# CVMethods/gabor_color_image_segmentation

Measured on AMD Instinct MI355X. Metric: Mpix/s segmented (Gabor+k-means), 481x321x3 batch, higher is better.
Workload: dtype i8; 1 GPU; batch 64/GPU synthetic 481x321x3 uint8 (seed 0), 4-scale x 6-orientation Gabor bank ksize 13 on a 2-level octave pyramid, k=8, n_iter=10; codebook=global, global_batch=64, parallelism=dp1 (images sharded, int64 centroid all-reduce)

## Files before the change

### gabor_color_image_segmentation_amd/_lib.py

```python
from __future__ import annotations

import ctypes as C
import os

_HERE = os.path.dirname(os.path.abspath(__file__))
LIB_PATH = os.environ.get("GCS_LIB_PATH") or os.path.join(_HERE, "csrc", "libgcs.so")

ABI_VERSION = 18
K_MAX = 16

_vp, _i, _sz = C.c_void_p, C.c_int, C.c_size_t

SIGNATURES = {
    "gcs_abi_version": (_i, []),
    "gcs_last_error": (C.c_char_p, []),
    "gcs_bank_packed_bytes": (_sz, [_i, _i]),
    "gcs_bank_bias_count": (_sz, [_i, _i]),
    "gcs_bank_pack": (_i, [_vp, _i, _i, _i, _vp, _vp]),
    "gcs_feature_slab_bytes": (_sz, [_i, _i, _i, _i, _i]),
    "gcs_feature_pass_bytes": (_sz, [_i, _i, _i, _i, _i]),
    "gcs_label_slab_bytes": (_sz, [_i, _i, _i]),
    "gcs_kmeans_parts_per_image": (_sz, [_i, _i, _i]),
    "gcs_kmeans_partial_bytes": (_sz, [_i, _i, _i, _i, _i]),
    "gcs_gabor_workspace_bytes": (_sz, [_i, _i, _i, _i]),
    "gcs_gabor_features": (_i, [_vp, _i, _i, _i, _vp, _vp, _i, _i, _i, _i, _vp, _vp, _vp]),
    "gcs_features_unpack": (_i, [_vp, _i, _i, _i, _i, _i, _vp, _vp]),
    "gcs_kmeans_init": (_i, [_vp, _i, _i, _i, _i, _i, _i, _i, _vp, _vp]),
    "gcs_features_gather": (_i, [_vp, _i, _i, _i, _i, _i, _i, _vp, _vp, _vp]),
    "gcs_kmeans_assign_accumulate": (_i, [_vp, _vp, _i, _i, _i, _i, _i, _i, _i, _i, _i, _i, _vp, _vp, _vp]),
    "gcs_kmeans_assign_raster": (_i, [_vp, _vp, _i, _i, _i, _i, _i, _i, _i, _i, _vp, _i, _vp, _vp]),
    "gcs_kmeans_reduce": (_i, [_vp, _i, _i, _i, _i, _i, _i, _vp, _vp]),
    "gcs_kmeans_finalize": (_i, [_vp, _i, _i, _i, _vp, _vp]),
    "gcs_kmeans_reduce_finalize": (_i, [_vp, _i, _i, _i, _i, _i, _i, _vp, _vp, _vp]),
    "gcs_download": (_i, [_vp, _vp, _sz, _vp]),
    "gcs_labels_widen": (_i, [_vp, _i, _i, _i, _vp, _vp]),
    "gcs_selftest_isqrt": (_i, [C.c_uint, _vp, _vp]),
    "gcs_selftest_native_parts": (_i, [_i, _i, _i]),
    "gcs_device_cu_count": (_i, []),
    "gcs_boundary_scratch_bytes": (_sz, [_i, _i, _i]),
    "gcs_boundary_counts": (_i, [_vp, _vp, _i, _i, _i, _vp, _vp, _vp]),
    "gcs_region_counts": (_i, [_vp, _vp, _i, _i, _i, _i, _i, _vp, _vp, _vp, _vp]),
    "gcs_boundary_batch_scratch_bytes": (_sz, [_i, _i, _i, _i]),
    "gcs_boundary_counts_batch": (_i, [_vp, _vp, _vp, _i, _i, _i, _i, _vp, _vp, _vp]),
    "gcs_region_counts_batch": (_i, [_vp, _vp, _vp, _i, _i, _i, _i, _i, _i, _i, _vp, _vp, _vp, _vp]),
    "gcs_region_counts_batch_u8": (_i, [_vp, _vp, _vp, _i, _i, _i, _i, _i, _i, _i, _vp, _vp, _vp, _vp]),
    "gcs_region_reduce": (_i, [_vp, _vp, _vp, _i, _i, _i, _vp, _vp, _vp]),
    "gcs_score_batch_resident": (_i, [_vp, _vp, _vp, _vp, _i, _vp, _vp, _i, _i, _i, _i, _i, _i, _i, _vp, _vp, _vp, _vp, _vp, _vp,
                                      _vp, _vp, _vp]),
# ... 49 lines not shown
```

### gabor_color_image_segmentation_amd/csrc/common.h

```cpp
#pragma once
#include <hip/hip_runtime.h>
#include <stdint.h>
#include <stdio.h>
#include <string.h>

#include "gcs.h"

typedef int v2i __attribute__((ext_vector_type(2)));
typedef int v4i __attribute__((ext_vector_type(4)));
typedef int v16i __attribute__((ext_vector_type(16)));

int gcs_fail(int code, const char *msg);
int gcs_hip_fail(hipError_t e, const char *what);
#define GCS_CHECK_LAUNCH(what)                               \
    do {                                                     \
        hipError_t e_ = hipGetLastError();                   \
        if (e_ != hipSuccess) return gcs_hip_fail(e_, what); \
    } while (0)

int gcs_cu_count();

static inline int round_up(int a, int m) { return (a + m - 1) / m * m; }
static inline int mtiles(int F) { return (F + 3) / 4; }

// ... 163 lines not shown
    const unsigned gi = slot % g, second = gi >= h ? 1u : 0u;
    byte = (slot / g) * h + gi - second * h;
    shift = 4 * (int)second;
}
__device__ __forceinline__ unsigned gcs_slab_value(const unsigned char *feats, const GcsLayout &lo, int b, int r, int y, int x) {
    if (!lo.split) return *reinterpret_cast<const uint16_t *>(feats + gcs_slab_offset(lo, b, r, y, x)) ^ 0x8080u;
    const unsigned char *img = feats + (size_t)b * lo.img_bytes;
    const unsigned slot = gcs_split_slot(lo, r, y, x);
    unsigned nb;
    int sh;
    gcs_split_nibble(gcs_level_of_plane(lo, r), slot, nb, sh);
    const unsigned lo8 = img[slot] ^ 0x80u, mid = (img[lo.mid_off + nb] >> sh) & 15u, top = (img[lo.top_off + nb] >> sh) & 15u;
    return lo8 | (mid << 8) | (top << 12);
}

constexpr int KP_PCH = 16;
__host__ __device__ __forceinline__ int partial_chunks(int row_len) { return (row_len + KP_PCH - 1) / KP_PCH; }
__device__ __forceinline__ size_t partial_index(int per_image, int b, int part, int parts, int nb, int i, int row_len) {
    const size_t rows = per_image ? (size_t)parts : (size_t)nb * parts;
    const size_t row = per_image ? (size_t)part : (size_t)b * parts + part;
    const size_t set = per_image ? (size_t)b : 0;
    return ((set * partial_chunks(row_len) + (size_t)(i / KP_PCH)) * rows + row) * KP_PCH + (size_t)(i % KP_PCH);
}
```

### gabor_color_image_segmentation_amd/csrc/kmeans.hip

```cpp
#include "common.h"
#include <type_traits>

#define LAYOUT_OR_FAIL(lo, who)                                        \
    GcsLayout lo;                                                      \
    if (B <= 0 || !gcs_make_layout(H, W, n_scales, n_orient, &lo))     \
        return gcs_fail(GCS_EINVAL, who ": bad shape or bank")

__global__ void kmeans_init_kernel(const unsigned char *__restrict__ feats, GcsLayout lo, int k,
                                   uint16_t *__restrict__ cent) {
    const int set = blockIdx.x;
    const long P = (long)lo.H * lo.W;
    for (int i = threadIdx.x; i < k * lo.D; i += blockDim.x) {
        const int j = i / lo.D, d = i % lo.D;
        const long p = ((2L * j + 1) * P) / (2L * k);
        const int y = (int)(p / lo.W), x = (int)(p % lo.W);
        cent[((size_t)set * k + j) * lo.D + d] = (uint16_t)gcs_slab_value(feats, lo, set, gcs_plane_of_logical(lo, d), y, x);
    }
}

extern "C" int gcs_kmeans_init(const uint16_t *feats, int B, int H, int W, int n_scales, int n_orient, int k,
                               int n_sets, uint16_t *cent, gcs_stream_t stream) {
    if (!feats || !cent) return gcs_fail(GCS_EINVAL, "gcs_kmeans_init: NULL pointer");
    LAYOUT_OR_FAIL(lo, "gcs_kmeans_init");
    if (k < 1 || k > GCS_K_MAX) return gcs_fail(GCS_EINVAL, "gcs_kmeans_init: k must be in 1..16");
// ... 205 lines not shown
    } while (0)
#define KP_PHASE_STORE                                                                                           \
    do {                                                                                                         \
        const int wg_ = (int)(blockIdx.y * gridDim.x + blockIdx.x);                                              \
        if (lane == 0 && wg_ < 1024) {                                                                           \
            for (int k_ = 0; k_ < 6; ++k_) g_kp_phases[(wg_ * 4 + (wid & 3)) * 8 + k_] = kp_ph[k_];             \
            g_kp_phases[(wg_ * 4 + (wid & 3)) * 8 + 6] = kp_tiles;                                               \
        }                                                                                                        \
    } while (0)
#else
#define KP_PHASE_DECL
#define KP_PHASE(k)
#define KP_PHASE_STORE
#endif

template <int KT, int NST, int DSTEPS, int WAVES, bool SPLIT = false, int L0T = 0>
__global__ __launch_bounds__(64 * WAVES, (WAVES == 8 ? 2
                                          : DSTEPS == KP_DSTEPS_NARROW && KT == 1 && NST <= (SPLIT ? 3 : 6) ? GCS_KP_WAVES
                                          : DSTEPS == KP_DSTEPS_NARROW ? 2 : 1)) void kmeans_pass_mfma_kernel(
    const unsigned char *__restrict__ feats, const uint16_t *__restrict__ cent, GcsLayout lo, int K, int per_image,
    int parts, int reverse, int row_lo, int row_hi, uint64_t *__restrict__ partials, void *__restrict__ raster,
    int raster_u8, int nt_flag) {
    constexpr int KP_ROWS = 16 * DSTEPS, KP_DSTEPS = DSTEPS, KP_NT = 2 * DSTEPS;
    constexpr int NTHR = 64 * WAVES;
    constexpr int NT_OWN = WAVES == 8 ? (KP_NT + 1) / 2 : KP_NT;
    constexpr int KP_COARSE = DSTEPS == KP_DSTEPS_NARROW ? 40 * 32 + 64 : 104 * 32 + 64;
    __shared__ __attribute__((aligned(16))) unsigned char s_tile[KP_ROWS * KP_PITCH];
    __shared__ __attribute__((aligned(16))) unsigned char s_coarse[KP_COARSE];
    __shared__ __attribute__((aligned(16))) unsigned char s_lab[KP_TP];
    __shared__ long long s_const[16];
    constexpr int KP_FLAGS = 320;
    __shared__ unsigned char s_flag[SPLIT ? KP_FLAGS : 4];
    static_assert(!SPLIT || (DSTEPS == KP_DSTEPS_NARROW && WAVES == 4), "the split slab is the narrow pass's");

    const bool do_acc = partials != nullptr;
    const int tid = threadIdx.x, lane = tid & 63;
    const int wid = tid >> 6;
    const int wave = wid & 3;
    const int half = wid >> 2;
    const int b = blockIdx.y, part = blockIdx.x;
    const int D = lo.D;
    const uint16_t *cset = cent + (size_t)(per_image ? b : 0) * K * D;
    const int ntiles = lo.ntiles;
    const int nimg = per_image ? 1 : (int)gridDim.y;
    const int G = parts * nimg, g = per_image ? part : b * parts + part;
    const int nlist = ntiles * nimg;
    const unsigned char *fb = feats + (size_t)(per_image ? b : 0) * lo.img_bytes;

    uint16_t *cs = reinterpret_cast<uint16_t *>(s_tile);
    for (int i = tid; i < 8 * KT * KP_ROWS; i += NTHR) {
        const int j = i / KP_ROWS, r = i % KP_ROWS;
        int e = 0;
        if (r >= lo.row0[0] && r < lo.row0[0] + lo.DL[0]) e = kp_logical_of<0>(lo, r - lo.row0[0]);
        if (lo.n_levels > 1 && r >= lo.row0[1] && r < lo.row0[1] + lo.DL[1]) e = kp_logical_of<1>(lo, r - lo.row0[1]);
        if (lo.n_levels > 2 && r >= lo.row0[2] && r < lo.row0[2] + lo.DL[2]) e = kp_logical_of<2>(lo, r - lo.row0[2]);
        if (lo.n_levels > 3 && r >= lo.row0[3] && r < lo.row0[3] + lo.DL[3]) e = kp_logical_of<3>(lo, r - lo.row0[3]);
        cs[i] = (j < K && r < D) ? (uint16_t)(cset[j * D + e] ^ 0x8080u) : (uint16_t)0;
    }
    if constexpr (SPLIT) {
        for (int it = tid; it < KP_FLAGS; it += NTHR) {
            const long long lt = (long long)g + (long long)it * G;
            unsigned char f = 0;
            if (lt < nlist) {
                const int T = reverse ? nlist - 1 - (int)lt : (int)lt;
// ... 539 lines not shown
            } else {
                bx -= dr;
                by -= dq;
                if (bx < 0) { bx += lo.bx_n; --by; }
            }
        }
        KP_PHASE(4);
        __syncthreads();
        KP_PHASE(5);
#ifdef GCS_KP_PHASES
        ++kp_tiles;
#endif
    }
    KP_PHASE_STORE;

    if (!do_acc) return;
    if constexpr (UPD2) {
        constexpr int RW2 = 16 * DSTEPS;
        int *red = reinterpret_cast<int *>(s_tile);
        static_assert(4 * 16 * RW2 * 4 <= KP_ROWS * KP_PITCH, "fold buffer exceeds the tile buffer");
#pragma unroll
        for (int pt = 0; pt < DSTEPS; ++pt)
#pragma unroll
            for (int e = 0; e < 4; ++e) red[(wave * 16 + 4 * ug + e) * RW2 + 16 * pt + un] = accu[pt][e];
        __syncthreads();
        const int D1 = D + 1;
        auto folded = [&](int j, int bb, int plane) {
            int sm_ = 0;
#pragma unroll
            for (int w = 0; w < 4; ++w) sm_ += red[(w * 16 + 2 * j + bb) * RW2 + plane];
            return -(long long)sm_ / 128;
        };
        for (int i = tid; i < K * D1; i += NTHR) {
            const int j = i / D1, e = i % D1;
            const long long nj = folded(j, 0, D);
            long long out = nj;
            if (e < D) {
                const int c = e / lo.F, f = e - c * lo.F;
                int pe = kp_plane_on_level<0>(lo, c, f);
                { const int q = kp_plane_on_level<1>(lo, c, f); pe = q >= 0 ? q : pe; }
                { const int q = kp_plane_on_level<2>(lo, c, f); pe = q >= 0 ? q : pe; }
                { const int q = kp_plane_on_level<3>(lo, c, f); pe = q >= 0 ? q : pe; }
                out = (folded(j, 0, pe) + 128 * nj) + 256 * (folded(j, 1, pe) + 128 * nj);
            }
            partials[partial_index(per_image, b, part, parts, (int)gridDim.y, i, K * D1)] = (uint64_t)out;
        }
    }
    if constexpr (!UPD2) {
    constexpr int RW = KP_NT * 16;
    int *red = reinterpret_cast<int *>(s_tile);
    static_assert(4 * 16 * RW * 4 <= KP_ROWS * KP_PITCH, "fold buffer exceeds the tile buffer");
#pragma unroll
    for (int nti = 0; nti < NT_OWN; ++nti) {
        const int nt = WAVES == 8 ? half * NT_OWN + nti : nti;
        if (nt < KP_NT)
#pragma unroll
            for (int e = 0; e < 4; ++e) red[(wave * 16 + 4 * ug + e) * RW + 16 * nt + un] = accu[nti][e];
    }
    __syncthreads();
// ... 538 lines not shown
    if (B > 65535) return gcs_fail(GCS_EINVAL, "gcs_kmeans_assign_accumulate: B too large for one launch");
    if ((long long)B * lo.ntiles > 0x1fffffffLL)
        return gcs_fail(GCS_EINVAL, "gcs_kmeans_assign_accumulate: batch too large for one launch");
    if (k < 1 || k > GCS_K_MAX) return gcs_fail(GCS_EINVAL, "gcs_kmeans_assign_accumulate: k must be in 1..16");
    if (n_sets != 1 && n_sets != B)
        return gcs_fail(GCS_EINVAL, "gcs_kmeans_assign_accumulate: n_sets must be 1 or B");
    const int D = lo.D;
    if (D < 16 * KP_DSTEPS_WIDE) {
        const int parts = (int)gcs_kmeans_parts_per_image(B, H, W);
        void *lab_out = raster ? raster : static_cast<void *>(labels);
        const int lab_u8 = raster ? raster_u8 : 1;
        const int nt_flag = 0;
#define GCS_KP_LAUNCHW(KT_, NST_, DS_, WV_)                                                                              \
    hipLaunchKernelGGL((kmeans_pass_mfma_kernel<KT_, NST_, DS_, WV_>), dim3(parts, B), dim3(64 * WV_), 0, stream,         \
                       reinterpret_cast<const unsigned char *>(feats), cent, lo, k, n_sets == B ? 1 : 0, parts,          \
                       reverse ? 1 : 0, row_lo, row_hi, partials, lab_out, lab_u8, nt_flag)
#define GCS_KP_LAUNCH(KT_, NST_, DS_) GCS_KP_LAUNCHW(KT_, NST_, DS_, 4)
        const int nchunk = lo.tile_bytes / 16;
        const int nst = (nchunk + 255) / 256;
        if (lo.split) {
            const int rounds = ((lo.S >> 4) + 255) / 256;
            const int nt_limit = kp_nt_limit(lo, B, n_sets, lo.tile_bytes / 4 * 3);
            if ((unsigned long long)lo.img_bytes >= (1ull << 32))
                return gcs_fail(GCS_EINVAL, "gcs_kmeans_assign_accumulate: image too large for the split slab's pass");
#define GCS_KP_LAUNCHS(KT_, NR_, ...)                                                                                          \
    hipLaunchKernelGGL((kmeans_pass_mfma_kernel<KT_, NR_, KP_DSTEPS_NARROW, 4, true __VA_OPT__(,) __VA_ARGS__>), dim3(parts, B), dim3(256), 0, stream, \
                       reinterpret_cast<const unsigned char *>(feats), cent, lo, k, n_sets == B ? 1 : 0, parts,             \
                       reverse ? 1 : 0, row_lo, row_hi, partials, lab_out, lab_u8, nt_limit)
            if (k <= 8 && rounds <= 3 && lo.DL[0] >= 32) { GCS_KP_LAUNCHS(1, 3, 2); }
            else if (k <= 8 && rounds <= 3) { GCS_KP_LAUNCHS(1, 3); }
            else if (k <= 8) { GCS_KP_LAUNCHS(1, 5); }
            else { GCS_KP_LAUNCHS(2, 5); }
#undef GCS_KP_LAUNCHS
        } else if (D < 16 * KP_DSTEPS_NARROW) {
            if (k <= 8) {
                if (nst <= 3) { GCS_KP_LAUNCH(1, 3, KP_DSTEPS_NARROW); }
                else if (nst <= 6) { GCS_KP_LAUNCH(1, 6, KP_DSTEPS_NARROW); }
                else if (nst <= 9) { GCS_KP_LAUNCH(1, 9, KP_DSTEPS_NARROW); }
                else { GCS_KP_LAUNCH(1, 10, KP_DSTEPS_NARROW); }
            } else {
                if (nst <= 6) { GCS_KP_LAUNCH(2, 6, KP_DSTEPS_NARROW); }
                else { GCS_KP_LAUNCH(2, 10, KP_DSTEPS_NARROW); }
            }
// ... 57 lines not shown
                                            int reverse, uint8_t *labels, uint64_t *partials, gcs_stream_t stream) {
    if (!labels && !partials)
        return gcs_fail(GCS_EINVAL, "gcs_kmeans_assign_accumulate: NULL pointer (labels and partials may not both be NULL)");
    return lloyd_pass(feats, cent, B, H, W, n_scales, n_orient, k, n_sets, row_lo, row_hi, reverse, labels, partials, nullptr, 0,
                      stream);
}

extern "C" int gcs_kmeans_assign_raster(const uint16_t *feats, const uint16_t *cent, int B, int H, int W, int n_scales,
                                        int n_orient, int k, int n_sets, int reverse, void *out, int out_u8,
                                        uint8_t *scratch_labels, gcs_stream_t stream) {
    if (!out) return gcs_fail(GCS_EINVAL, "gcs_kmeans_assign_raster: NULL pointer");
    return lloyd_pass(feats, cent, B, H, W, n_scales, n_orient, k, n_sets, 0, H, reverse, scratch_labels, nullptr, out,
                      out_u8 ? 1 : 0, stream);
}

template <bool FIN, int RG>
__global__ __launch_bounds__(16 * RG) void kmeans_reduce_kernel(const uint64_t *__restrict__ partials,
                                                             int rows_per_set, int row_len, int D1,
                                                             long long *__restrict__ sums,
                                                             uint16_t *__restrict__ cent) {
    __shared__ unsigned long long sm_s[RG][KP_PCH], sm_c[RG][KP_PCH];
    const int set = blockIdx.y, chunk = blockIdx.x, t = threadIdx.x;
    const int e16 = t & (KP_PCH - 1), rg = t >> 4;
    const int nch = partial_chunks(row_len);
    const int e = chunk * KP_PCH + e16;
    const int ee = e < row_len ? e : row_len - 1;
    const int j = ee / D1, d = ee - j * D1;
    const int ec = j * D1 + (D1 - 1);
    const uint64_t *p = partials + (((size_t)set * nch + chunk) * rows_per_set) * KP_PCH + (ee - chunk * KP_PCH);
    const uint64_t *pc = partials + (((size_t)set * nch + ec / KP_PCH) * rows_per_set) * KP_PCH + ec % KP_PCH;
// ... 134 lines not shown
```

### gabor_color_image_segmentation_amd/segmenter.py

```python
from __future__ import annotations

import math
import os

import numpy as np

from . import _lib
from .bank import GaborBank, check_color_weight, make_bank, smoothing_taps

_SLAB_BUDGET = 16 << 30
_GRAPH_MAX_PIXELS = 1 << 20


class DebugSwitches:

    def __init__(self, spec=""):
        self.no_reverse = self.no_graph = self.force_collectives = False
        self.slab_candidates = None
        for item in filter(None, (x.strip() for x in spec.split(","))):
            name, _, val = item.partition("=")
            if name == "slab_candidates" and val.isdigit():
                self.slab_candidates = int(val)
            elif name in ("no_reverse", "no_graph", "force_collectives") and not val:
                setattr(self, name, True)
# ... 112 lines not shown
        packed = np.zeros(self.lib.gcs_bank_packed_bytes(ns, no), np.int8)
        bias = np.zeros(self.lib.gcs_bank_bias_count(ns, no), np.int32)
        tapq = np.ascontiguousarray(bank.tapq, np.int16)
        _lib.check(self.lib.gcs_bank_pack(tapq.ctypes.data, ns, no, bank.ksize, packed.ctypes.data,
                                          bias.ctypes.data), "gcs_bank_pack")
        self.packed = torch.from_numpy(packed).to(self.device)
        self.bias = torch.from_numpy(bias).to(self.device)
        self._gabor_ws = None
        self.chroma_gain = _check_chroma_gain(chroma_gain)
        self.smoothing = _check_smoothing(smoothing, bank)
        self._smooth_ws = self.smooth_taps = self.smooth_radius = None
        if self.smoothing > 0:
            taps, radius = smoothing_taps(self.smoothing, ns, no, bank.f_max, bank.ratio)
            self.smooth_taps = torch.from_numpy(taps).to(self.device)
            self.smooth_radius = torch.from_numpy(radius).to(self.device)

    def empty_bytes(self, n):
        return self.torch.empty(int(n), dtype=self.torch.uint8, device=self.device)

    def feature_slab(self, b, h, w):
        return self.empty_bytes(self.lib.gcs_feature_slab_bytes(b, h, w, *self._bk))

    def label_slab(self, b, h, w):
        return self.empty_bytes(self.lib.gcs_label_slab_bytes(b, h, w))

    def partial_slab(self, b, h, w, k):
        return self.empty_bytes(self.lib.gcs_kmeans_partial_bytes(b, h, w, self.bank.n_features, k))

    def _stream(self):
        return self.torch.cuda.current_stream(self.device).cuda_stream

    def _check_dev(self, *tensors):
        for t in tensors:
            if t.device != self.device:
                raise ValueError(f"tensor on {t.device}, this Segmenter's kernels run on {self.device}")

    def gabor_scratch(self, b, h, w):
        return self.empty_bytes(self.lib.gcs_gabor_workspace_bytes(b, h, w, self.bank.n_scales))

    @_on_device
    def gabor_features(self, imgs, feats, scratch=None):
        b, h, w, _ = imgs.shape
# ... 43 lines not shown
                   "gcs_smooth_features")

    @_on_device
    def features_unpack(self, feats, b, h, w):
        d = self.bank.n_features
        out = self.torch.empty((b, d, h, w), dtype=self.torch.int16, device=self.device)
        _lib.check(self.lib.gcs_features_unpack(feats.data_ptr(), b, h, w, *self._bk, out.data_ptr(),
                                                self._stream()), "gcs_features_unpack")
        return out

    @_on_device
    def kmeans_init(self, feats, b, h, w, k, n_sets, cent):
        _lib.check(self.lib.gcs_kmeans_init(feats.data_ptr(), b, h, w, *self._bk, k, n_sets,
                                            cent.data_ptr(), self._stream()), "gcs_kmeans_init")

    @_on_device
    def assign_accumulate(self, feats, cent, b, h, w, k, n_sets, labels, partials, rows=None, reverse=False):
        lo, hi = rows if rows is not None else (0, h)
        _lib.check(self.lib.gcs_kmeans_assign_accumulate(
            feats.data_ptr(), cent.data_ptr(), b, h, w, *self._bk, k, n_sets, lo, hi,
            1 if reverse else 0, None if labels is None else labels.data_ptr(),
            None if partials is None else partials.data_ptr(), self._stream()),
            "gcs_kmeans_assign_accumulate")

    @_on_device
    def assign_raster(self, feats, cent, b, h, w, k, n_sets, out, scratch_labels=None, reverse=False):
        torch = self.torch
        if out.dtype not in (torch.int32, torch.uint8) or tuple(out.shape) != (b, h, w) or not out.is_contiguous():
            raise ValueError("out must be a contiguous (B,H,W) int32 or uint8 tensor")
        _lib.check(self.lib.gcs_kmeans_assign_raster(
            feats.data_ptr(), cent.data_ptr(), b, h, w, *self._bk, k, n_sets, 1 if reverse else 0, out.data_ptr(),
            1 if out.dtype == torch.uint8 else 0, None if scratch_labels is None else scratch_labels.data_ptr(),
            self._stream()), "gcs_kmeans_assign_raster")

    def download(self, dst_pinned, src):
        self._check_dev(src)
        n = src.numel() * src.element_size()
        if not dst_pinned.is_pinned() or dst_pinned.numel() * dst_pinned.element_size() != n \
                or not src.is_contiguous() or not dst_pinned.is_contiguous():
            raise ValueError("download needs a contiguous device tensor and a pinned host tensor of the same size")
        with self.torch.cuda.device(self.device):
            _lib.check(self.lib.gcs_download(src.data_ptr(), dst_pinned.data_ptr(), n, self._stream()), "gcs_download")

    @_on_device
# ... 70 lines not shown


def _check_smoothing(smoothing, bank) -> float:
    try:
        K = float(smoothing)
    except (TypeError, ValueError):
        raise ValueError(f"smoothing must be a number, got {smoothing!r}") from None
    if not math.isfinite(K) or K < 0.0:
        raise ValueError(f"smoothing must be finite and >= 0, got {smoothing!r}")
    if K > 0.0:
        smoothing_taps(K, bank.n_scales, bank.n_orient, bank.f_max, bank.ratio)
    return K


def lloyd(ops, feats, b, h, w, k, n_iter, mode, labels, partials, cent, sums, dist_group=None,
          rows=None, init=None, raster=None, debug=_ENV_DEBUG):
    n_sets = b if mode == "per_image" else 1
    dist = None
    if mode == "global":
        import torch.distributed as td
        if td.is_available() and td.is_initialized() and (td.get_world_size(dist_group) > 1 or debug.force_collectives):
            dist = td
    if init is not None:
        init(cent)
    else:
        ops.kmeans_init(feats, b, h, w, k, n_sets, cent)
        if dist is not None:
            _collective(dist.broadcast, cent.view(_torch().uint8),
                        src=dist.get_global_rank(dist_group, 0) if dist_group is not None else 0,
                        group=dist_group)
    for t in range(n_iter):
        last = t == n_iter - 1
        rev = not (t & 1) and not debug.no_reverse
        if last and raster is not None:
            ops.assign_raster(feats, cent, b, h, w, k, n_sets, raster, scratch_labels=labels, reverse=rev)
            break
        ops.assign_accumulate(feats, cent, b, h, w, k, n_sets, labels if last else None, None if last else partials, rows,
# ... 68 lines not shown
        except Exception:
            pass

    @property
    def native(self):
        return hasattr(self.ops, "lib")

    def _workspace(self, g, h, w, mode):
        key = (g, h, w, mode)
        ws = self._ws.get(key)
        if ws is None:
            n_sets = g if mode == "per_image" else 1
            ws = dict(feats=self.ops.feature_slab(g, h, w), labels=self.ops.label_slab(g, h, w),
                      partials=self.ops.partial_slab(g, h, w, self.k),
                      cent=self.ops.new_centroids(n_sets, self.k), sums=self.ops.new_sums(n_sets, self.k))
            if self.smoothing > 0:
                ws["smooth"] = self.ops.smooth_scratch(g, h, w)
            if self.chroma_gain > 0:
                ws["colour"] = self.ops.colour_scratch(g, h, w)
            self._place_slab(ws, g, h, w, n_sets)
            if len(self._ws) >= 8:
                self._ws.pop(next(iter(self._ws)))
            self._ws[key] = ws
        return ws

    def _place_slab(self, ws, g, h, w, n_sets):
        n_cand = self.slab_candidates
        if not self.native or ws["feats"].numel() < (256 << 20) or n_cand <= 1:
            return
        torch = _torch()
# ... 48 lines not shown
            raise ValueError(f"imgs live on {imgs.device}, this Segmenter on {self.ops.device}")
        if out is None:
            out = torch.empty((b, h, w), dtype=torch.int32, device=imgs.device)
        elif out.dtype != torch.int32 or tuple(out.shape) != (b, h, w) or out.device != imgs.device \
                or not out.is_contiguous():
            raise ValueError("out must be a contiguous (B,H,W) int32 tensor on the device of imgs")
        g = group or self.group_size(b, h, w, mode)
        import contextlib
        with (torch.cuda.device(self.ops.device) if on_gpu else contextlib.nullcontext()):
            for g0 in range(0, b, g):
                n = min(g, b - g0)
                ws = self._workspace(n, h, w, mode) if n == g else self._tail_workspace(n, h, w, mode)
                self._features(imgs[g0:g0 + n], ws, n, h, w)
                direct = hasattr(self.ops, "assign_raster")
                lloyd(self.ops, ws["feats"], n, h, w, self.k, self.n_iter, mode, ws["labels"], ws["partials"],
                      ws["cent"], ws["sums"], dist_group, raster=out[g0:g0 + n] if direct else None, debug=self.debug)
                if not direct:
                    self.ops.labels_widen(ws["labels"], n, h, w, out[g0:g0 + n])
            if self.min_region_size > 0:
                regions = torch.empty_like(out)
                self.ops.merge_small_regions(out, self.min_region_size, regions)
                out.copy_(regions)
            elif self.connectivity:
                regions = torch.empty_like(out)
                self.ops.connected_regions(out, regions)
                out.copy_(regions)
        return out

    def _tail_workspace(self, n, h, w, mode):
        n_sets = n if mode == "per_image" else 1
        ws = dict(feats=self.ops.feature_slab(n, h, w), labels=self.ops.label_slab(n, h, w),
                  partials=self.ops.partial_slab(n, h, w, self.k),
                  cent=self.ops.new_centroids(n_sets, self.k), sums=self.ops.new_sums(n_sets, self.k))
        if self.smoothing > 0:
            ws["smooth"] = self.ops.smooth_scratch(n, h, w)
        if self.chroma_gain > 0:
            ws["colour"] = self.ops.colour_scratch(n, h, w)
        return ws

    def _features(self, imgs, ws, b, h, w):
        self.ops.gabor_features(self._opponent(imgs, ws["colour"]) if self.chroma_gain > 0 else imgs, ws["feats"])
        if self.smoothing > 0:
            self.ops.smooth_features(ws["feats"], b, h, w, scratch=ws["smooth"])

    def _opponent(self, imgs, colour):
        self.ops.colour_opponent(imgs, colour)
        return colour

# ... 150 lines not shown
            for i in range(n_chunks):
                g0, g1 = bounds[i], bounds[i + 1]
                staged[i].result()
                with torch.cuda.stream(st["copy"]):
                    st["dev_in"][g0:g1].copy_(st["pin_in"][g0:g1], non_blocking=True)
                    st["ev"][i].record(st["copy"])
                cur.wait_event(st["ev"][i])
                chunk = st["dev_in"][g0:g1]
                if self.chroma_gain > 0:
                    chunk = self._opponent(chunk, ws["colour"][g0:g1])
                ops.gabor_features(chunk, ws["feats"][g0 * per_img:])
            if self.smoothing > 0:
                ops.smooth_features(ws["feats"], b, h, w, scratch=ws["smooth"])
            dev_out = st["dev_out"] if out_dtype == np.uint8 else st["dev_out32"]
            lloyd(ops, ws["feats"], b, h, w, self.k, self.n_iter, mode, ws["labels"], ws["partials"],
                  ws["cent"], ws["sums"], raster=dev_out, debug=self.debug)
            res = torch.empty((b, h, w), dtype=dev_out.dtype, pin_memory=True)
            ops.download(res, dev_out)
            cur.synchronize()
        return res.numpy()

    def segment_stream(self, batches, mode="per_image", out_dtype=np.int32, depth=2):
        out_dtype = np.dtype(out_dtype)
        if out_dtype not in (np.dtype(np.int32), np.dtype(np.uint8)):
            raise ValueError("out_dtype must be int32 or uint8")
        if mode not in ("per_image", "global"):
            raise ValueError("mode must be 'per_image' or 'global'")
        dist_on = False
        if mode == "global":
            import torch.distributed as td
            dist_on = td.is_available() and td.is_initialized()
# ... 22 lines not shown
                dev_out = torch.empty((b, h, w), dtype=torch.uint8 if out_dtype == np.uint8 else torch.int32, device=dev)
                pin_in = torch.empty((b, h, w, 3), dtype=torch.uint8, pin_memory=True)
                scratch = self.ops.gabor_scratch(b, h, w)
                smooth = ws.get("smooth")
                colour = ws.get("colour")

                ops, k, n_iter, debug = self.ops, self.k, self.n_iter, self.debug

                def step():
                    if colour is not None:
                        ops.colour_opponent(dev_in, colour)
                    ops.gabor_features(dev_in if colour is None else colour, ws["feats"], scratch=scratch)
                    if smooth is not None:
                        ops.smooth_features(ws["feats"], b, h, w, scratch=smooth)
                    lloyd(ops, ws["feats"], b, h, w, k, n_iter, mode, ws["labels"], ws["partials"], ws["cent"],
                          ws["sums"], raster=dev_out, debug=debug)
                dev_in.zero_()
                step()
                torch.cuda.current_stream(dev).synchronize()
                graph = torch.cuda.CUDAGraph()
                if not _CAPTURES.capture(torch, graph, step, dev):
                    _CAPTURES.fell_back(key, "torch.cuda.graph raised RuntimeError")
                    graph = None
                    torch.cuda.current_stream(dev).synchronize()
                ent = dict(graph=graph, step=step, ws=ws, dev_in=dev_in, dev_out=dev_out, pin_in=pin_in, scratch=scratch)
                if len(self._graphs) >= 4:
                    _CAPTURES.retire([self._graphs.pop(next(iter(self._graphs)))])
                self._graphs[key] = ent
            cur = torch.cuda.current_stream(dev)
            _stage(ent["pin_in"], imgs)
            ent["dev_in"].copy_(ent["pin_in"], non_blocking=True)
# ... 162 lines not shown
                st["ev_up"][i].synchronize()
            _stage(st["pin_in"][i], imgs)
            with torch.cuda.stream(st["up"]):
                if n >= n_slots:
                    st["up"].wait_event(st["ev_done"][i])
                st["dev_in"][i].copy_(st["pin_in"][i], non_blocking=True)
                st["ev_up"][i].record(st["up"])
            cur.wait_event(st["ev_up"][i])
            if n >= n_slots:
                cur.wait_event(st["ev_down"][i])
            ops.gabor_features(seg._opponent(st["dev_in"][i], ws["colour"]) if seg.chroma_gain > 0 else st["dev_in"][i],
                               ws["feats"])
            if seg.smoothing > 0:
                ops.smooth_features(ws["feats"], b, h, w, scratch=ws["smooth"])
            lloyd(ops, ws["feats"], b, h, w, seg.k, seg.n_iter, self.mode, ws["labels"], ws["partials"], ws["cent"],
                  ws["sums"], raster=st["dev_out"][i], debug=seg.debug)
            st["ev_done"][i].record(cur)
            land = torch.empty((b, h, w), dtype=self.t_dtype, pin_memory=True)
            with torch.cuda.stream(st["down"]):
                st["down"].wait_event(st["ev_done"][i])
                ops.download(land, st["dev_out"][i])
                st["ev_down"][i].record(st["down"])
            ev = torch.cuda.Event()
            ev.record(st["down"])
            self.pending.append((ev, land.numpy()))
            self.n += 1
            out = []
            while len(self.pending) > self.depth:
                ev0, res0 = self.pending.pop(0)
                ev0.synchronize()
                out.append(res0)
# ... 75 lines not shown
```

### include/gcs.h

```cpp
#ifndef GCS_H
#define GCS_H

#include <stddef.h>
#include <stdint.h>

#ifdef __cplusplus
extern "C" {
#endif

typedef struct ihipStream_t *gcs_stream_t;

enum {
    GCS_OK = 0,
    GCS_EINVAL = 1,
    GCS_EHIP = 2
};

#define GCS_ABI_VERSION 18
#define GCS_KSIZE_MAX 15
#define GCS_K_MAX 16
#define GCS_TAP_ABS_SUM_MAX 32896
#define GCS_SCALES_MAX 8

int gcs_abi_version(void);
// ... 38 lines not shown

int gcs_kmeans_assign_raster(const uint16_t *feats_dev, const uint16_t *centroids_dev, int B, int H, int W, int n_scales,
                             int n_orient, int k, int n_sets, int reverse, void *out_dev, int out_u8,
                             uint8_t *scratch_labels_dev, gcs_stream_t stream);

int gcs_kmeans_reduce(const uint64_t *partials_dev, int B, int H, int W, int D, int k, int n_sets,
                      int64_t *sums_dev, gcs_stream_t stream);

int gcs_kmeans_finalize(const int64_t *sums_dev, int n_sets, int k, int D,
                        uint16_t *centroids_dev, gcs_stream_t stream);

int gcs_kmeans_reduce_finalize(const uint64_t *partials_dev, int B, int H, int W, int D, int k,
                               int n_sets, int64_t *sums_dev, uint16_t *centroids_dev,
                               gcs_stream_t stream);

int gcs_labels_widen(const uint8_t *labels_dev, int B, int H, int W, int32_t *out_dev,
                     gcs_stream_t stream);

int gcs_selftest_isqrt(unsigned n_max, unsigned *bad_dev, gcs_stream_t stream);
int gcs_selftest_native_parts(int B, int H, int W);


size_t gcs_boundary_scratch_bytes(int A, int H, int W);
int gcs_boundary_counts(const int32_t *labels_dev, const uint16_t *truth_dev, int A, int H, int W,
                        void *scratch_dev, uint64_t *counts_dev, gcs_stream_t stream);

size_t gcs_boundary_batch_scratch_bytes(int B, int T, int H, int W);
int gcs_boundary_counts_batch(const int32_t *labels_dev, const uint16_t *truth_dev, const int32_t *img_of_dev, int B, int T,
                              int H, int W, void *scratch_dev, uint64_t *counts_dev, gcs_stream_t stream);

// ... 59 lines not shown
```

Before: 5460 Mpix/s.

## Fuse k-means centroid update into the assign pass with atomic fold rows

Adds a self-updating k-means pass. Each launch recomputes the centroids from the previous pass's atomically folded sums (or seeds them on pass 0), assigns pixels, and atomically adds its partial sums into a rotating triple-buffered workspace. A ticket counter lets the last workgroup clear the previous buffer. This removes the separate reduce/finalize launches and the per-part partial slab traffic per Lloyd iteration. The cost is that every workgroup redundantly re-folds the sums, and it relies on global atomics and ticket ordering.

```diff
diff --git a/gabor_color_image_segmentation_amd/_lib.py b/gabor_color_image_segmentation_amd/_lib.py
--- a/gabor_color_image_segmentation_amd/_lib.py
+++ b/gabor_color_image_segmentation_amd/_lib.py
@@ -32,6 +32,8 @@
     "gcs_kmeans_reduce": (_i, [_vp, _i, _i, _i, _i, _i, _i, _vp, _vp]),
     "gcs_kmeans_finalize": (_i, [_vp, _i, _i, _i, _vp, _vp]),
     "gcs_kmeans_reduce_finalize": (_i, [_vp, _i, _i, _i, _i, _i, _i, _vp, _vp, _vp]),
+    "gcs_kmeans_fused_workspace_bytes": (_sz, [_i, _i, _i, _i, _i, _i, _i]),
+    "gcs_kmeans_pass_fused": (_i, [_vp, _i, _i, _i, _i, _i, _i, _i, _i, _i, _i, _vp, _vp, _vp, _i, _vp]),
     "gcs_download": (_i, [_vp, _vp, _sz, _vp]),
     "gcs_labels_widen": (_i, [_vp, _i, _i, _i, _vp, _vp]),
     "gcs_selftest_isqrt": (_i, [C.c_uint, _vp, _vp]),
diff --git a/gabor_color_image_segmentation_amd/csrc/common.h b/gabor_color_image_segmentation_amd/csrc/common.h
--- a/gabor_color_image_segmentation_amd/csrc/common.h
+++ b/gabor_color_image_segmentation_amd/csrc/common.h
@@ -201,6 +201,14 @@
     return lo8 | (mid << 8) | (top << 12);
 }
 
+struct GcsFold {
+    unsigned long long *prev;
+    unsigned long long *clear;
+    uint16_t *cent_new;
+    uint16_t *cent_out;
+    unsigned *ticket;
+    int rows;
+};
 constexpr int KP_PCH = 16;
 __host__ __device__ __forceinline__ int partial_chunks(int row_len) { return (row_len + KP_PCH - 1) / KP_PCH; }
 __device__ __forceinline__ size_t partial_index(int per_image, int b, int part, int parts, int nb, int i, int row_len) {
diff --git a/gabor_color_image_segmentation_amd/csrc/kmeans.hip b/gabor_color_image_segmentation_amd/csrc/kmeans.hip
--- a/gabor_color_image_segmentation_amd/csrc/kmeans.hip
+++ b/gabor_color_image_segmentation_amd/csrc/kmeans.hip
@@ -1,4 +1,5 @@
 #include "common.h"
+#include <stdlib.h>
 #include <type_traits>
 
 #define LAYOUT_OR_FAIL(lo, who)                                        \
@@ -243,13 +244,13 @@
 #define KP_PHASE_STORE
 #endif
 
-template <int KT, int NST, int DSTEPS, int WAVES, bool SPLIT = false, int L0T = 0>
+template <int KT, int NST, int DSTEPS, int WAVES, bool SPLIT = false, int L0T = 0, bool FUSED = false>
 __global__ __launch_bounds__(64 * WAVES, (WAVES == 8 ? 2
                                           : DSTEPS == KP_DSTEPS_NARROW && KT == 1 && NST <= (SPLIT ? 3 : 6) ? GCS_KP_WAVES
                                           : DSTEPS == KP_DSTEPS_NARROW ? 2 : 1)) void kmeans_pass_mfma_kernel(
     const unsigned char *__restrict__ feats, const uint16_t *__restrict__ cent, GcsLayout lo, int K, int per_image,
     int parts, int reverse, int row_lo, int row_hi, uint64_t *__restrict__ partials, void *__restrict__ raster,
-    int raster_u8, int nt_flag) {
+    int raster_u8, int nt_flag, GcsFold fz) {
     constexpr int KP_ROWS = 16 * DSTEPS, KP_DSTEPS = DSTEPS, KP_NT = 2 * DSTEPS;
     constexpr int NTHR = 64 * WAVES;
     constexpr int NT_OWN = WAVES == 8 ? (KP_NT + 1) / 2 : KP_NT;
@@ -261,6 +262,7 @@
     constexpr int KP_FLAGS = 320;
     __shared__ unsigned char s_flag[SPLIT ? KP_FLAGS : 4];
     static_assert(!SPLIT || (DSTEPS == KP_DSTEPS_NARROW && WAVES == 4), "the split slab is the narrow pass's");
+    static_assert(!FUSED || (SPLIT && KT == 1), "the self-updating pass exists for the CL1 kernels");
 
     const bool do_acc = partials != nullptr;
     const int tid = threadIdx.x, lane = tid & 63;
@@ -277,6 +279,52 @@
     const unsigned char *fb = feats + (size_t)(per_image ? b : 0) * lo.img_bytes;
 
     uint16_t *cs = reinterpret_cast<uint16_t *>(s_tile);
+    if constexpr (FUSED) {
+        const int D1 = D + 1, row_len = K * D1;
+        const int set = per_image ? b : 0;
+        const int wg = b * (int)gridDim.x + part, nwg = (int)(gridDim.x * gridDim.y);
+        {
+            const long long total = (long long)(per_image ? (int)gridDim.y : 1) * fz.rows * row_len;
+            for (long long i = (long long)wg * NTHR + tid; i < total; i += (long long)nwg * NTHR) fz.clear[i] = 0ull;
+        }
+        unsigned long long *fsum = reinterpret_cast<unsigned long long *>(s_tile + 8 * KT * KP_ROWS * 2);
+        static_assert(8 * KT * KP_ROWS * 2 % 16 == 0 && 8 * KT * KP_ROWS * 2 + 8 * (8 * KT * KP_ROWS) <= KP_ROWS * KP_PITCH,
+                      "the folded sums do not fit behind the centroid scratch");
+        const bool later = fz.prev != nullptr;
+        if (later) {
+            const unsigned long long *pv = fz.prev + (size_t)set * fz.rows * row_len;
+            for (int i = tid; i < row_len; i += NTHR) {
+                unsigned long long s = 0;
+                for (int r = 0; r < fz.rows; ++r) s += pv[(size_t)r * row_len + i];
+                fsum[i] = s;
+            }
+            __syncthreads();
+        }
+        const bool writer = part == 0 && (per_image || b == 0);
+        const long long P = (long long)lo.H * lo.W;
+        for (int i = tid; i < 8 * KT * KP_ROWS; i += NTHR) {
+            const int j = i / KP_ROWS, r = i % KP_ROWS;
+            int e = 0;
+            if (r >= lo.row0[0] && r < lo.row0[0] + lo.DL[0]) e = kp_logical_of<0>(lo, r - lo.row0[0]);
+            if (lo.n_levels > 1 && r >= lo.row0[1] && r < lo.row0[1] + lo.DL[1]) e = kp_logical_of<1>(lo, r - lo.row0[1]);
+            unsigned v = 0;
+            if (j < K && r < D) {
+                if (later) {
+                    const unsigned long long c = fsum[j * D1 + D], s = fsum[j * D1 + e];
+                    v = c > 0 ? (unsigned)((2 * s + c) / (2 * c)) : (unsigned)cset[j * D + e];
+                } else {
+                    const long long p = ((2LL * j + 1) * P) / (2LL * K);
+                    v = gcs_slab_value(feats, lo, set, r, (int)(p / lo.W), (int)(p % lo.W));
+                }
+                if (writer) {
+                    fz.cent_new[((size_t)set * K + j) * D + e] = (uint16_t)v;
+                    fz.cent_out[((size_t)set * K + j) * D + e] = (uint16_t)v;
+                }
+                v ^= 0x8080u;
+            }
+            cs[i] = (uint16_t)v;
+        }
+    } else
     for (int i = tid; i < 8 * KT * KP_ROWS; i += NTHR) {
         const int j = i / KP_ROWS, r = i % KP_ROWS;
         int e = 0;
@@ -846,6 +894,19 @@
     }
     KP_PHASE_STORE;
 
+    if constexpr (FUSED) {
+        if (!do_acc && fz.prev != nullptr) {
+            __shared__ int s_last;
+            const int nwg = (int)(gridDim.x * gridDim.y);
+            if (tid == 0) s_last = atomicAdd(fz.ticket, 1u) == (unsigned)(nwg - 1);
+            __syncthreads();
+            if (s_last) {
+                const long long total = (long long)(per_image ? (int)gridDim.y : 1) * fz.rows * K * (D + 1);
+                for (long long i = tid; i < total; i += NTHR) fz.prev[i] = 0ull;
+                if (tid == 0) *fz.ticket = 0u;
+            }
+        }
+    }
     if (!do_acc) return;
     if constexpr (UPD2) {
         constexpr int RW2 = 16 * DSTEPS;
@@ -875,6 +936,12 @@
                 { const int q = kp_plane_on_level<3>(lo, c, f); pe = q >= 0 ? q : pe; }
                 out = (folded(j, 0, pe) + 128 * nj) + 256 * (folded(j, 1, pe) + 128 * nj);
             }
+            if constexpr (FUSED) {
+                const int wg = b * (int)gridDim.x + part;
+                unsigned long long *row = reinterpret_cast<unsigned long long *>(partials) +
+                                          ((size_t)(per_image ? b : 0) * fz.rows + (size_t)(wg % fz.rows)) * (K * D1);
+                if (out != 0) atomicAdd(&row[i], (unsigned long long)out);
+            } else
             partials[partial_index(per_image, b, part, parts, (int)gridDim.y, i, K * D1)] = (uint64_t)out;
         }
     }
@@ -1443,7 +1510,7 @@
 #define GCS_KP_LAUNCHW(KT_, NST_, DS_, WV_)                                                                              \
     hipLaunchKernelGGL((kmeans_pass_mfma_kernel<KT_, NST_, DS_, WV_>), dim3(parts, B), dim3(64 * WV_), 0, stream,         \
                        reinterpret_cast<const unsigned char *>(feats), cent, lo, k, n_sets == B ? 1 : 0, parts,          \
-                       reverse ? 1 : 0, row_lo, row_hi, partials, lab_out, lab_u8, nt_flag)
+                       reverse ? 1 : 0, row_lo, row_hi, partials, lab_out, lab_u8, nt_flag, GcsFold{})
 #define GCS_KP_LAUNCH(KT_, NST_, DS_) GCS_KP_LAUNCHW(KT_, NST_, DS_, 4)
         const int nchunk = lo.tile_bytes / 16;
         const int nst = (nchunk + 255) / 256;
@@ -1455,7 +1522,7 @@
 #define GCS_KP_LAUNCHS(KT_, NR_, ...)                                                                                          \
     hipLaunchKernelGGL((kmeans_pass_mfma_kernel<KT_, NR_, KP_DSTEPS_NARROW, 4, true __VA_OPT__(,) __VA_ARGS__>), dim3(parts, B), dim3(256), 0, stream, \
                        reinterpret_cast<const unsigned char *>(feats), cent, lo, k, n_sets == B ? 1 : 0, parts,             \
-                       reverse ? 1 : 0, row_lo, row_hi, partials, lab_out, lab_u8, nt_limit)
+                       reverse ? 1 : 0, row_lo, row_hi, partials, lab_out, lab_u8, nt_limit, GcsFold{})
             if (k <= 8 && rounds <= 3 && lo.DL[0] >= 32) { GCS_KP_LAUNCHS(1, 3, 2); }
             else if (k <= 8 && rounds <= 3) { GCS_KP_LAUNCHS(1, 3); }
             else if (k <= 8) { GCS_KP_LAUNCHS(1, 5); }
@@ -1543,6 +1610,73 @@
                       out_u8 ? 1 : 0, stream);
 }
 
+#ifndef KP_FOLD_ROWS
+#define KP_FOLD_ROWS 1
+#endif
+static int fold_rows(int B, int parts, int n_sets) {
+    if (n_sets == B && B > 1) return 1;
+    static const int env = [] {
+        const char *e = getenv("GCS_KP_FOLD_ROWS");
+        const int v = e ? atoi(e) : 0;
+        return v >= 1 && v <= 64 ? v : KP_FOLD_ROWS;
+    }();
+    const long long wgs = (long long)B * parts;
+    return (int)(wgs < env ? wgs : env);
+}
+static bool fused_bank(const GcsLayout &lo, int k) {
+    return lo.split && k >= 1 && k <= 8 && ((lo.S >> 4) + 255) / 256 <= 3;
+}
+static size_t fused_sum_bytes(const GcsLayout &lo, int k, int n_sets, int rows) {
+    return ((size_t)n_sets * rows * k * (lo.D + 1) * 8 + 255) & ~(size_t)255;
+}
+static size_t fused_cent_bytes(const GcsLayout &lo, int k, int n_sets) {
+    return ((size_t)n_sets * k * lo.D * 2 + 255) & ~(size_t)255;
+}
+extern "C" size_t gcs_kmeans_fused_workspace_bytes(int B, int H, int W, int n_scales, int n_orient, int k, int n_sets) {
+    GcsLayout lo;
+    if (B <= 0 || B > 65535 || !gcs_make_layout(H, W, n_scales, n_orient, &lo) || (n_sets != 1 && n_sets != B) || !fused_bank(lo, k))
+        return 0;
+    const int rows = fold_rows(B, (int)gcs_kmeans_parts_per_image(B, H, W), n_sets);
+    return 3 * fused_sum_bytes(lo, k, n_sets, rows) + 2 * fused_cent_bytes(lo, k, n_sets) + 256;
+}
+
+extern "C" int gcs_kmeans_pass_fused(const uint16_t *feats, int B, int H, int W, int n_scales, int n_orient, int k, int n_sets,
+                                     int reverse, int pass, int last, void *workspace, uint16_t *cent, void *out, int out_u8,
+                                     gcs_stream_t stream) {
+    if (!feats || !workspace || !cent || (last && !out))
+        return gcs_fail(GCS_EINVAL, "gcs_kmeans_pass_fused: NULL pointer (the last pass needs its label map)");
+    LAYOUT_OR_FAIL(lo, "gcs_kmeans_pass_fused");
+    if (pass < 0) return gcs_fail(GCS_EINVAL, "gcs_kmeans_pass_fused: pass must be >= 0");
+    if (gcs_kmeans_fused_workspace_bytes(B, H, W, n_scales, n_orient, k, n_sets) == 0)
+        return gcs_fail(GCS_EINVAL, "gcs_kmeans_pass_fused: no self-updating pass for this bank / k / n_sets (gcs_kmeans_fused_workspace_bytes == 0)");
+    if ((long long)B * lo.ntiles > 0x1fffffffLL || (unsigned long long)lo.img_bytes >= (1ull << 32))
+        return gcs_fail(GCS_EINVAL, "gcs_kmeans_pass_fused: batch or image too large for one launch");
+    const int parts = (int)gcs_kmeans_parts_per_image(B, H, W);
+    const int rows = fold_rows(B, parts, n_sets);
+    const size_t sb = fused_sum_bytes(lo, k, n_sets, rows), cb = fused_cent_bytes(lo, k, n_sets);
+    unsigned char *ws = static_cast<unsigned char *>(workspace);
+    auto sums = [&](int t) { return reinterpret_cast<unsigned long long *>(ws + (size_t)(t % 3) * sb); };
+    auto cents = [&](int t) { return reinterpret_cast<uint16_t *>(ws + 3 * sb + (size_t)(t & 1) * cb); };
+    GcsFold fz;
+    fz.prev = pass > 0 ? sums(pass - 1) : nullptr;
+    fz.clear = sums(pass + 1);
+    fz.cent_new = cents(pass);
+    fz.cent_out = cent;
+    fz.ticket = reinterpret_cast<unsigned *>(ws + 3 * sb + 2 * cb);
+    fz.rows = rows;
+    uint64_t *acc = last ? nullptr : reinterpret_cast<uint64_t *>(sums(pass));
+    const int nt_limit = kp_nt_limit(lo, B, n_sets, lo.tile_bytes / 4 * 3);
+#define GCS_KP_LAUNCHF(L0T_)                                                                                                   \
+    hipLaunchKernelGGL((kmeans_pass_mfma_kernel<1, 3, KP_DSTEPS_NARROW, 4, true, L0T_, true>), dim3(parts, B), dim3(256), 0, stream, \
+                       reinterpret_cast<const unsigned char *>(feats), cents(pass + 1), lo, k, n_sets == B ? 1 : 0, parts,     \
+                       reverse ? 1 : 0, 0, H, acc, last ? out : nullptr, out_u8 ? 1 : 0, nt_limit, fz)
+    if (lo.DL[0] >= 32) { GCS_KP_LAUNCHF(2); }
+    else { GCS_KP_LAUNCHF(0); }
+#undef GCS_KP_LAUNCHF
+    GCS_CHECK_LAUNCH("gcs_kmeans_pass_fused");
+    return GCS_OK;
+}
+
 template <bool FIN, int RG>
 __global__ __launch_bounds__(16 * RG) void kmeans_reduce_kernel(const uint64_t *__restrict__ partials,
                                                              int rows_per_set, int row_len, int D1,
diff --git a/gabor_color_image_segmentation_amd/segmenter.py b/gabor_color_image_segmentation_amd/segmenter.py
--- a/gabor_color_image_segmentation_amd/segmenter.py
+++ b/gabor_color_image_segmentation_amd/segmenter.py
@@ -150,6 +150,8 @@
             taps, radius = smoothing_taps(self.smoothing, ns, no, bank.f_max, bank.ratio)
             self.smooth_taps = torch.from_numpy(taps).to(self.device)
             self.smooth_radius = torch.from_numpy(radius).to(self.device)
+        self.has_fused = all(n in _lib.SIGNATURES and hasattr(self.lib, n)
+                             for n in ("gcs_kmeans_fused_workspace_bytes", "gcs_kmeans_pass_fused"))
 
     def empty_bytes(self, n):
         return self.torch.empty(int(n), dtype=self.torch.uint8, device=self.device)
@@ -162,6 +164,10 @@
 
     def partial_slab(self, b, h, w, k):
         return self.empty_bytes(self.lib.gcs_kmeans_partial_bytes(b, h, w, self.bank.n_features, k))
+
+    def fused_workspace(self, b, h, w, k, n_sets):
+        n = self.lib.gcs_kmeans_fused_workspace_bytes(b, h, w, *self._bk, k, n_sets) if self.has_fused else 0
+        return self.torch.zeros(int(n), dtype=self.torch.uint8, device=self.device) if n else None
 
     def _stream(self):
         return self.torch.cuda.current_stream(self.device).cuda_stream
@@ -235,8 +241,20 @@
         _lib.check(self.lib.gcs_kmeans_init(feats.data_ptr(), b, h, w, *self._bk, k, n_sets,
                                             cent.data_ptr(), self._stream()), "gcs_kmeans_init")
 
-    @_on_device
-    def assign_accumulate(self, feats, cent, b, h, w, k, n_sets, labels, partials, rows=None, reverse=False):
+    def _pass_fused(self, feats, cent, b, h, w, k, n_sets, fused, reverse, out=None):
+        fold, t = fused
+        self._check_dev(fold)
+        _lib.check(self.lib.gcs_kmeans_pass_fused(
+            feats.data_ptr(), b, h, w, *self._bk, k, n_sets, 1 if reverse else 0, t, 0 if out is None else 1,
+            fold.data_ptr(), cent.data_ptr(), None if out is None else out.data_ptr(),
+            1 if out is not None and out.dtype == self.torch.uint8 else 0, self._stream()), "gcs_kmeans_pass_fused")
+
+    @_on_device
+    def assign_accumulate(self, feats, cent, b, h, w, k, n_sets, labels, partials, rows=None, reverse=False, fused=None):
+        if fused is not None:
+            if labels is not None or partials is not None or rows is not None:
+                raise ValueError("a self-updating pass takes whole images and has no label or partial output")
+            return self._pass_fused(feats, cent, b, h, w, k, n_sets, fused, reverse)
         lo, hi = rows if rows is not None else (0, h)
         _lib.check(self.lib.gcs_kmeans_assign_accumulate(
             feats.data_ptr(), cent.data_ptr(), b, h, w, *self._bk, k, n_sets, lo, hi,
@@ -245,10 +263,12 @@
             "gcs_kmeans_assign_accumulate")
 
     @_on_device
-    def assign_raster(self, feats, cent, b, h, w, k, n_sets, out, scratch_labels=None, reverse=False):
+    def assign_raster(self, feats, cent, b, h, w, k, n_sets, out, scratch_labels=None, reverse=False, fused=None):
         torch = self.torch
         if out.dtype not in (torch.int32, torch.uint8) or tuple(out.shape) != (b, h, w) or not out.is_contiguous():
             raise ValueError("out must be a contiguous (B,H,W) int32 or uint8 tensor")
+        if fused is not None:
+            return self._pass_fused(feats, cent, b, h, w, k, n_sets, fused, reverse, out=out)
         _lib.check(self.lib.gcs_kmeans_assign_raster(
             feats.data_ptr(), cent.data_ptr(), b, h, w, *self._bk, k, n_sets, 1 if reverse else 0, out.data_ptr(),
             1 if out.dtype == torch.uint8 else 0, None if scratch_labels is None else scratch_labels.data_ptr(),
@@ -349,13 +369,21 @@
 
 
 def lloyd(ops, feats, b, h, w, k, n_iter, mode, labels, partials, cent, sums, dist_group=None,
-          rows=None, init=None, raster=None, debug=_ENV_DEBUG):
+          rows=None, init=None, raster=None, debug=_ENV_DEBUG, fold=None):
     n_sets = b if mode == "per_image" else 1
     dist = None
     if mode == "global":
         import torch.distributed as td
         if td.is_available() and td.is_initialized() and (td.get_world_size(dist_group) > 1 or debug.force_collectives):
             dist = td
+    if fold is not None and dist is None and rows is None and init is None and raster is not None and n_iter >= 1:
+        for t in range(n_iter):
+            rev = not (t & 1) and not debug.no_reverse
+            if t == n_iter - 1:
+                ops.assign_raster(feats, cent, b, h, w, k, n_sets, raster, scratch_labels=labels, reverse=rev, fused=(fold, t))
+            else:
+                ops.assign_accumulate(feats, cent, b, h, w, k, n_sets, None, None, reverse=rev, fused=(fold, t))
+        return
     if init is not None:
         init(cent)
     else:
@@ -454,6 +482,8 @@
             ws = dict(feats=self.ops.feature_slab(g, h, w), labels=self.ops.label_slab(g, h, w),
                       partials=self.ops.partial_slab(g, h, w, self.k),
                       cent=self.ops.new_centroids(n_sets, self.k), sums=self.ops.new_sums(n_sets, self.k))
+            if hasattr(self.ops, "fused_workspace"):
+                ws["fold"] = self.ops.fused_workspace(g, h, w, self.k, n_sets)
             if self.smoothing > 0:
                 ws["smooth"] = self.ops.smooth_scratch(g, h, w)
             if self.chroma_gain > 0:
@@ -532,7 +562,8 @@
                 self._features(imgs[g0:g0 + n], ws, n, h, w)
                 direct = hasattr(self.ops, "assign_raster")
                 lloyd(self.ops, ws["feats"], n, h, w, self.k, self.n_iter, mode, ws["labels"], ws["partials"],
-                      ws["cent"], ws["sums"], dist_group, raster=out[g0:g0 + n] if direct else None, debug=self.debug)
+                      ws["cent"], ws["sums"], dist_group, raster=out[g0:g0 + n] if direct else None, debug=self.debug,
+                      fold=ws.get("fold"))
                 if not direct:
                     self.ops.labels_widen(ws["labels"], n, h, w, out[g0:g0 + n])
             if self.min_region_size > 0:
@@ -550,6 +581,8 @@
         ws = dict(feats=self.ops.feature_slab(n, h, w), labels=self.ops.label_slab(n, h, w),
                   partials=self.ops.partial_slab(n, h, w, self.k),
                   cent=self.ops.new_centroids(n_sets, self.k), sums=self.ops.new_sums(n_sets, self.k))
+        if hasattr(self.ops, "fused_workspace"):
+            ws["fold"] = self.ops.fused_workspace(n, h, w, self.k, n_sets)
         if self.smoothing > 0:
             ws["smooth"] = self.ops.smooth_scratch(n, h, w)
         if self.chroma_gain > 0:
@@ -730,7 +763,7 @@
                 ops.smooth_features(ws["feats"], b, h, w, scratch=ws["smooth"])
             dev_out = st["dev_out"] if out_dtype == np.uint8 else st["dev_out32"]
             lloyd(ops, ws["feats"], b, h, w, self.k, self.n_iter, mode, ws["labels"], ws["partials"],
-                  ws["cent"], ws["sums"], raster=dev_out, debug=self.debug)
+                  ws["cent"], ws["sums"], raster=dev_out, debug=self.debug, fold=ws.get("fold"))
             res = torch.empty((b, h, w), dtype=dev_out.dtype, pin_memory=True)
             ops.download(res, dev_out)
             cur.synchronize()
@@ -783,7 +816,7 @@
                     if smooth is not None:
                         ops.smooth_features(ws["feats"], b, h, w, scratch=smooth)
                     lloyd(ops, ws["feats"], b, h, w, k, n_iter, mode, ws["labels"], ws["partials"], ws["cent"],
-                          ws["sums"], raster=dev_out, debug=debug)
+                          ws["sums"], raster=dev_out, debug=debug, fold=ws.get("fold"))
                 dev_in.zero_()
                 step()
                 torch.cuda.current_stream(dev).synchronize()
@@ -976,7 +1009,7 @@
             if seg.smoothing > 0:
                 ops.smooth_features(ws["feats"], b, h, w, scratch=ws["smooth"])
             lloyd(ops, ws["feats"], b, h, w, seg.k, seg.n_iter, self.mode, ws["labels"], ws["partials"], ws["cent"],
-                  ws["sums"], raster=st["dev_out"][i], debug=seg.debug)
+                  ws["sums"], raster=st["dev_out"][i], debug=seg.debug, fold=ws.get("fold"))
             st["ev_done"][i].record(cur)
             land = torch.empty((b, h, w), dtype=self.t_dtype, pin_memory=True)
             with torch.cuda.stream(st["down"]):
diff --git a/include/gcs.h b/include/gcs.h
--- a/include/gcs.h
+++ b/include/gcs.h
@@ -76,6 +76,11 @@
                                int n_sets, int64_t *sums_dev, uint16_t *centroids_dev,
                                gcs_stream_t stream);
 
+size_t gcs_kmeans_fused_workspace_bytes(int B, int H, int W, int n_scales, int n_orient, int k, int n_sets);
+int gcs_kmeans_pass_fused(const uint16_t *feats_dev, int B, int H, int W, int n_scales, int n_orient, int k, int n_sets,
+                          int reverse, int pass, int last, void *workspace_dev, uint16_t *centroids_dev, void *out_dev,
+                          int out_u8, gcs_stream_t stream);
+
 int gcs_labels_widen(const uint8_t *labels_dev, int B, int H, int W, int32_t *out_dev,
                      gcs_stream_t stream);
 
```

After: 5586 Mpix/s, median of 6. 1.02x the previous value.
